# faltiska/Matcha-TTS-24k

Measured on AMD Instinct MI355X. Metric: mel-frames/s (100-bin, 24 kHz) end-to-end synthesise(), n_timesteps=10, higher is better.
Workload: dtype f32 via 2-term f16 split (fp32 accumulate)

## Files before the change

### include/mtts.h

```cpp
#ifndef MTTS_H
#define MTTS_H

#include <stddef.h>
#include <stdint.h>

#ifdef __cplusplus
extern "C" {
#endif

#define MTTS_ABI_VERSION 2
#define MTTS_IMAGE_REVISION 5

typedef struct mtts_ctx mtts_ctx;

typedef struct mtts_config {
    int32_t n_feats;
    int32_t n_spks;
    int32_t spk_emb_dim;
    int32_t n_vocab;
    int32_t enc_channels;
    int32_t enc_filter;
    int32_t enc_heads;
    int32_t enc_layers;
    int32_t enc_kernel;
// ... 60 lines not shown

int mtts_fold_rows(mtts_ctx* ctx, int y_max, int align);
int mtts_cfm_solve_folded(mtts_ctx* ctx, const float* d_x0, const float* d_mu, const int64_t* d_y_lengths, int y_max, int add_mu,
                          const float* h_t_span, int n_steps, int solver, int B, int T, int T_fold, float* d_out, int T_out,
                          float out_scale, float out_shift, void* d_ws, int64_t ws_bytes, void* stream);


int64_t mtts_gemm_packed_bytes(int N, int C, int ntaps);
int mtts_gemm_f32(const float* d_a, int lda, int B, int T_in, int C, int ntaps, const int* h_tap_off, int in_stride,
                  int T_out, const float* d_a_mask, const float* d_a_mean, const float* d_a_rstd, const float* d_a_part,
                  int a_nparts, const float* d_w,
                  void* d_wpacked, const float* d_bias, int N, int act, const float* d_p0, const float* d_p1,
                  const float* d_res, int ldr, const float* d_out_mask, float out_scale, float* d_out, int ldc,
                  float* d_stats_out, int terms, void* stream);

int64_t mtts_gemm_p16_scratch_bytes(int B, int T_in, int C, int T_out, int N);
int mtts_gemm_p16(const float* d_a, int lda, int B, int T_in, int C, int ntaps, const int* h_tap_off, int in_stride, int T_out,
                  const float* d_a_mask, const float* d_a_mean, const float* d_a_rstd, const float* d_a_part, int a_nparts,
                  const float* d_w, void* d_wpacked, const float* d_bias, int N, int act, const float* d_p0, const float* d_p1,
                  const float* d_res, int ldr, const float* d_out_mask, float out_scale, float* d_out, int ldc,
                  float* d_out16_f32, float out_lscale, float* d_stats_out, int force_bm, void* d_scratch, void* stream);

int64_t mtts_conv_gn_scratch_bytes(int B, int T, int C, int N);
int mtts_conv_gn(const float* d_x, int B, int T, int C, int c1, const float* d_w, void* d_wpacked, const float* d_bias, int N,
                 const float* d_gamma, const float* d_beta, const float* d_mask, const float* d_chbias, const int* d_nrows,
                 const int* d_nextra, const float* d_bias_stats, float eps, float* d_out, void* d_scratch, void* stream);

int mtts_attention_f32(const float* d_qkv, const float* d_mask, int B, int T, int H, int D, float scale, int mask_mode,
                       float* d_out, void* stream);

int mtts_attention_p16(const float* d_qkv, const float* d_mask, int B, int T, int H, int D, float scale, int mask_mode,
                       float* d_out, void* d_scratch, void* stream);

int64_t mtts_chain_stream_frags(int C, int inner, int ch, int n_qkv);
int mtts_chain_plan(int M, int ch, int* qb, int* prefetch_wgs);
int mtts_chain_stream_pack(int C, int inner, int ch, int n_qkv, const float* h_w_out, const float* h_w1, const float* h_w2,
                           const float* h_w_qkv, uint16_t* h_dst);
int64_t mtts_chain_stream_frags_pair(int C, int inner, int ch, int n_qkv);
int mtts_chain_stream_pack_pair(int C, int inner, int ch, int n_qkv, const float* h_w_out, const float* h_w1, const float* h_w2,
                                const float* h_w_qkv, uint16_t* h_dst);
int64_t mtts_tblock_chain_scratch_bytes(int M, int C, int inner, int n_qkv, int ch);
int mtts_tblock_chain(const float* d_att, const float* d_x, int M, int C, int inner, const float* h_w_out, const float* h_b_out,
                      const float* h_w1, const float* h_b1, const float* h_p0, const float* h_p1, const float* h_w2,
                      const float* h_b2, const float* h_w_qkv, const float* h_b_qkv, int n_qkv, const float* d_out_mask, int qb,
                      int ch, float* d_x_out, float* d_qkv_out, void* d_scratch, void* stream);
int mtts_tblock_chain_timed(const float* d_att, const float* d_x, int M, int C, int inner, const float* h_w_out, const float* h_b_out,
                            const float* h_w1, const float* h_b1, const float* h_p0, const float* h_p1, const float* h_w2,
                            const float* h_b2, const float* h_w_qkv, const float* h_b_qkv, int n_qkv, const float* d_out_mask,
                            int qb, int ch, float* d_x_out, float* d_qkv_out, void* d_scratch, void* stream, int repeat, float* h_ms);
int mtts_tblock_chain_pair_timed(const float* d_att, const float* d_x, int M, int C, int inner, const float* h_w_out, const float* h_b_out,
                                 const float* h_w1, const float* h_b1, const float* h_p0, const float* h_p1, const float* h_w2,
                                 const float* h_b2, const float* h_w_qkv, const float* h_b_qkv, int n_qkv, const float* d_out_mask,
                                 int qb, int ch, float* d_x_out, float* d_qkv_out, void* d_scratch, void* stream, int repeat, float* h_ms);

int mtts_row_stats(const float* d_x, int M, int C, int ld, float eps, float* d_mean, float* d_rstd, void* stream);

int mtts_channel_layernorm(const float* d_x, int B, int T, int C, const float* d_gamma, const float* d_beta, float eps, int act,
                           const float* d_film, const float* d_mask, float* d_y, void* stream);

int64_t mtts_groupnorm_scratch_bytes(int B, int T, int G);
int mtts_groupnorm_mish(const float* d_y, const float* d_gamma, const float* d_beta, const float* d_mask, int B, int T,
                        int C, int G, float eps, float* d_out, void* d_scratch, void* stream);


typedef struct mtts_vocos mtts_vocos;
mtts_vocos* mtts_vocos_create(int n_mels, int dim, int intermediate_dim, int num_layers, int n_fft, int hop_length);
// ... 26 lines not shown
```

### matcha-tts-24k_amd/_hip.py

```python
from __future__ import annotations

import ctypes as C
import os
import subprocess
from pathlib import Path
from typing import Dict, Optional

import numpy as np
import torch

from .hparams import PathHParams

HERE = Path(__file__).resolve().parent
CSRC = HERE / "csrc"
LIB = Path(os.environ["MTTS_HIP_LIB"]) if os.environ.get("MTTS_HIP_LIB") else HERE / "libmtts_hip.so"
SOURCES = ["gemm_f32.hip", "attention_f32.hip", "gemm_p16.hip", "tblock_chain.hip", "resnet_conv.hip", "norm_glue.hip", "vocos.hip", "model.hip"]
HEADERS = [CSRC / "kernels.h", CSRC / "device_utils.h", CSRC / "model.h", HERE.parent / "include" / "mtts.h"]
SOLVERS = {"euler": 0, "midpoint": 1, "rk4": 2}


class MttsConfig(C.Structure):
    _fields_ = [(n, C.c_int32) for n in (
        "n_feats", "n_spks", "spk_emb_dim", "n_vocab", "enc_channels", "enc_filter", "enc_heads", "enc_layers",
        "enc_kernel", "prenet_layers", "prenet_kernel", "dp_filter", "dp_kernel", "dp_layers", "dec_levels")] + [
        ("dec_channels", C.c_int32 * 4)] + [(n, C.c_int32) for n in (
            "dec_head_dim", "dec_heads", "dec_n_blocks", "dec_mid_blocks")]


def _deps(src: Path, seen=None):
    import re
    seen = set() if seen is None else seen
    if src in seen or not src.exists():
        return seen
    seen.add(src)
    for inc in re.findall(r'^\s*#\s*include\s+"([^"]+)"', src.read_text(), flags=re.M):
        _deps((src.parent / inc).resolve(), seen)
    return seen


BUILD_MODE = "not built in this process"


def build(force: bool = False, verbose: bool = False) -> Path:
    global BUILD_MODE
    srcs = [CSRC / s for s in SOURCES]
    if LIB.exists() and not force:
        deps = set(HEADERS)
        for src in srcs:
            deps |= _deps(src.resolve())
# ... 44 lines not shown
    if _lib is not None:
        return _lib
    if not LIB.exists():
        raise RuntimeError(f"{LIB} is missing: run `python -c 'import __graft_entry__ as g; g.build()'` "
                           "(the HIP path has no CPU fallback)")
    lib = C.CDLL(str(LIB))
    vp, i32, i64, f32 = C.c_void_p, C.c_int, C.c_int64, C.c_float
    sig = {
        "mtts_abi_version": (i32, []),
        "mtts_last_error": (C.c_char_p, []),
        "mtts_create": (vp, [C.POINTER(MttsConfig)]),
        "mtts_destroy": (None, [vp]),
        "mtts_set_tensor": (i32, [vp, C.c_char_p, vp, i64]),
        "mtts_weights_bytes": (i64, [vp]),
        "mtts_upload_weights": (i32, [vp, vp, i64]),
        "mtts_debug_hold": (i32, [vp, i32]),
        "mtts_weights_signature": (i32, [vp, C.c_char_p, i64]),
        "mtts_export_weights": (i32, [vp, vp, i64, C.POINTER(i32)]),
        "mtts_import_weights": (i32, [vp, vp, i64, i32]),
        "mtts_encoder_workspace_bytes": (i64, [vp, i32, i32]),
        "mtts_text_encoder_forward": (i32, [vp, vp, vp, vp, vp, i32, i32, vp, vp, vp, vp, i64, vp]),
        "mtts_speaker_embedding": (i32, [vp, i32, vp, i32, vp, vp]),
        "mtts_durations": (i32, [vp, vp, f32, f32, i32, i32, vp, vp, vp, vp]),
        "mtts_durations_per_utterance": (i32, [vp, vp, vp, vp, i32, i32, vp, vp, vp, vp]),
        "mtts_align_pool": (i32, [vp, vp, vp, i32, i32, i32, i32, vp, vp, vp, vp]),
        "mtts_set_frame_limits": (i32, [vp, vp]),
        "mtts_decoder_workspace_bytes": (i64, [vp, i32, i32]),
        "mtts_decoder_forward": (i32, [vp, vp, vp, vp, f32, i32, i32, vp, vp, i64, vp]),
        "mtts_cfm_solve": (i32, [vp, vp, vp, vp, i32, vp, i32, i32, i32, i32, vp, i32, f32, f32, vp, i64, vp]),
        "mtts_fold_rows": (i32, [vp, i32, i32]),
        "mtts_cfm_solve_folded": (i32, [vp, vp, vp, vp, i32, i32, vp, i32, i32, i32, i32, i32, vp, i32, f32, f32, vp, i64, vp]),
        "mtts_gemm_packed_bytes": (i64, [i32, i32, i32]),
        "mtts_attention_p16": (i32, [vp, vp, i32, i32, i32, i32, f32, i32, vp, vp, vp]),
        "mtts_gemm_p16_scratch_bytes": (i64, [i32, i32, i32, i32, i32]),
        "mtts_conv_gn_scratch_bytes": (i64, [i32, i32, i32, i32]),
        "mtts_conv_gn": (i32, [vp, i32, i32, i32, i32, vp, vp, vp, i32, vp, vp, vp, vp, vp, vp, vp, f32, vp, vp, vp]),
        "mtts_gemm_p16": (i32, [vp, i32, i32, i32, i32, i32, vp, i32, i32, vp, vp, vp, vp, i32, vp, vp, vp, i32, i32, vp, vp, vp,
                                i32, vp, f32, vp, i32, vp, f32, vp, i32, vp, vp]),
        "mtts_gemm_f32": (i32, [vp, i32, i32, i32, i32, i32, vp, i32, i32, vp, vp, vp, vp, i32, vp, vp, vp, i32, i32, vp, vp, vp,
                                i32, vp, f32, vp, i32, vp, i32, vp]),
        "mtts_attention_f32": (i32, [vp, vp, i32, i32, i32, i32, f32, i32, vp, vp]),
        "mtts_chain_stream_frags": (i64, [i32, i32, i32, i32]),
        "mtts_chain_plan": (i32, [i32, i32, C.POINTER(C.c_int), C.POINTER(C.c_int)]),
        "mtts_chain_stream_frags_pair": (i64, [i32, i32, i32, i32]),
        "mtts_chain_stream_pack_pair": (i32, [i32, i32, i32, i32, vp, vp, vp, vp, vp]),
        "mtts_chain_stream_pack": (i32, [i32, i32, i32, i32, vp, vp, vp, vp, vp]),
        "mtts_tblock_chain_scratch_bytes": (i64, [i32, i32, i32, i32, i32]),
        "mtts_tblock_chain": (i32, [vp, vp, i32, i32, i32, vp, vp, vp, vp, vp, vp, vp, vp, vp, vp, i32, vp, i32, i32, vp, vp, vp, vp]),
        "mtts_tblock_chain_timed": (i32, [vp, vp, i32, i32, i32, vp, vp, vp, vp, vp, vp, vp, vp, vp, vp, i32, vp, i32, i32, vp, vp, vp, vp,
                                          i32, C.POINTER(C.c_float)]),
        "mtts_tblock_chain_pair_timed": (i32, [vp, vp, i32, i32, i32, vp, vp, vp, vp, vp, vp, vp, vp, vp, vp, i32, vp, i32, i32, vp, vp, vp, vp,
                                          i32, C.POINTER(C.c_float)]),
        "mtts_row_stats": (i32, [vp, i32, i32, i32, f32, vp, vp, vp]),
        "mtts_channel_layernorm": (i32, [vp, i32, i32, i32, vp, vp, f32, i32, vp, vp, vp, vp]),
        "mtts_groupnorm_scratch_bytes": (i64, [i32, i32, i32]),
        "mtts_groupnorm_mish": (i32, [vp, vp, vp, vp, i32, i32, i32, i32, f32, vp, vp, vp]),
        "mtts_vocos_create": (vp, [i32, i32, i32, i32, i32, i32]),
        "mtts_vocos_destroy": (None, [vp]),
        "mtts_vocos_set_tensor": (i32, [vp, C.c_char_p, vp, i64]),
        "mtts_vocos_weights_bytes": (i64, [vp]),
        "mtts_vocos_upload_weights": (i32, [vp, vp, i64]),
        "mtts_vocos_workspace_bytes": (i64, [vp, i32, i32]),
        "mtts_vocos_decode": (i32, [vp, vp, i32, i32, vp, vp, i64, vp]),
        "mtts_gemm_terms": (i32, [vp]),
        "mtts_set_arithmetic": (i32, [vp, i32]),
        "mtts_weights_saturate": (i32, [vp]),
# ... 389 lines not shown
    n = lib.mtts_tblock_chain_scratch_bytes(M, Cc, inner, n_qkv, ch)
    if n < 0:
        raise RuntimeError("mtts_tblock_chain: unsupported shape")
    scratch = torch.empty(n, dtype=torch.uint8, device=x.device)
    x_out = torch.empty(M, Cc, dtype=torch.float32, device=x.device)
    qkv = torch.empty(M, n_qkv, dtype=torch.float32, device=x.device) if n_qkv else None
    keep = [_host(t) for t in (w_out, b_out, w1, b1, p0, p1, w2, b2, w_qkv, b_qkv)]
    hp = [k[1] for k in keep]
    ms = C.c_float(0.0)
    check((lib.mtts_tblock_chain_pair_timed if pair else lib.mtts_tblock_chain_timed)(ptr(att), ptr(x), M, Cc, inner, hp[0], hp[1], hp[2], hp[3], hp[4], hp[5], hp[6], hp[7], hp[8], hp[9],
                                      n_qkv, ptr(out_mask), qb, ch, ptr(x_out), ptr(qkv), scratch.data_ptr(), stream_ptr(), repeat,
                                      C.byref(ms)))
    torch.cuda.synchronize()
    if repeat:
        return x_out, qkv, ms.value
    return x_out, qkv


def attention_f32(qkv, mask, B, T, H, D, scale, mask_mode):
    lib = load()
    out = torch.empty(B * T, H * D, dtype=torch.float32, device=qkv.device)
    check(lib.mtts_attention_f32(ptr(qkv), ptr(mask), B, T, H, D, float(scale), mask_mode, ptr(out), stream_ptr()))
    return out


def attention_p16(qkv, mask, B, T, H, D, scale, mask_mode):
    lib = load()
    out = torch.empty(B * T, H * D, dtype=torch.float32, device=qkv.device)
    scratch = torch.empty(16 * B * T * H * D, dtype=torch.uint8, device=qkv.device)
    check(lib.mtts_attention_p16(ptr(qkv), ptr(mask), B, T, H, D, float(scale), mask_mode, ptr(out), scratch.data_ptr(), stream_ptr()))
    return out


def row_stats(x, eps=1e-5):
    lib = load()
    M, Cc = x.shape
    mean = torch.empty(M, dtype=torch.float32, device=x.device)
    rstd = torch.empty(M, dtype=torch.float32, device=x.device)
    check(lib.mtts_row_stats(ptr(x), M, Cc, Cc, eps, ptr(mean), ptr(rstd), stream_ptr()))
    return mean, rstd


def channel_layernorm(x, gamma, beta, B, T, *, act=0, film=None, mask=None, eps=1e-5):
    lib = load()
    y = torch.empty_like(x)
    check(lib.mtts_channel_layernorm(ptr(x), B, T, x.shape[1], ptr(gamma), ptr(beta), float(eps), act, ptr(film), ptr(mask), ptr(y),
                                     stream_ptr()))
    return y


def groupnorm_mish(y, gamma, beta, mask, B, T, G=8, eps=1e-5):
    lib = load()
    Cc = y.shape[1]
    scratch = torch.empty(lib.mtts_groupnorm_scratch_bytes(B, T, G), dtype=torch.uint8, device=y.device)
    out = torch.empty_like(y)
    check(lib.mtts_groupnorm_mish(ptr(y), ptr(gamma), ptr(beta), ptr(mask), B, T, Cc, G, eps, ptr(out), scratch.data_ptr(),
                                  stream_ptr()))
    return out
```

### matcha-tts-24k_amd/csrc/attention_f32.hip

```cpp
#include "kernels.h"
#include "device_utils.h"
#include <cstdlib>
#include <string>

namespace mtts {

using f32x16 = __attribute__((ext_vector_type(16))) float;
using f32x4 = __attribute__((ext_vector_type(4))) float;
using f16x8 = __attribute__((ext_vector_type(8))) _Float16;
using f16x4 = __attribute__((ext_vector_type(4))) _Float16;

constexpr int AT_QW = 32;
constexpr int AT_K = 64;
constexpr int AT_D = 64;
constexpr int AT_KS = 72;
constexpr float NEG_BIG = -1e30f;
constexpr float LOG2E = 1.44269504088896340736f;

__device__ __forceinline__ f16x4 tr_read4(const _Float16* lds_ptr) {
    typedef __fp16 h4 __attribute__((__vector_size__(4 * sizeof(__fp16))));
    const h4 v = __builtin_amdgcn_ds_read_tr16_b64_v4f16((__attribute__((address_space(3))) h4*)(lds_ptr));
    return __builtin_bit_cast(f16x4, v);
}

// ... 294 lines not shown
                        *reinterpret_cast<f16x4*>(op + t * 32 + 8 * g4 + 4 * h) = hh;
                    } else {
                        *reinterpret_cast<f16x4*>(op + t * 64 + 8 * g4 + 4 * h) = hh;
                        *reinterpret_cast<f16x4*>(op + t * 64 + 32 + 8 * g4 + 4 * h) = ll;
                    }
                }
        }
        raise_range_flag(p.range_flag, range_bad);
    } else if (q_in) {
        float* op = p.out + (rowbase + qi) * (size_t)(p.H * p.D) + head * p.D;
#pragma unroll
        for (int t = 0; t < 2; ++t)
#pragma unroll
            for (int g4 = 0; g4 < 4; ++g4) {
                const int d = 32 * t + 8 * g4 + 4 * h;
                if (d < p.D) {
                    f32x4 v = {o[t][4 * g4] * inv, o[t][4 * g4 + 1] * inv, o[t][4 * g4 + 2] * inv, o[t][4 * g4 + 3] * inv};
                    *reinterpret_cast<f32x4*>(op + d) = v;
                }
            }
    }
}

hipError_t launch_attention(const AttnArgs& a, hipStream_t s) {
    const bool p16 = a.qkv16 != nullptr;
    const int ew = a.half16 ? 1 : 2;
    if ((a.half16 && !p16) || (a.bf16 && !a.half16)) return hipErrorInvalidValue;
    if (p16 ? (!a.out16 || a.D != AT_D || a.ld16 < 3 * ew * a.H * AT_D || (a.ld16 & 7) || a.ldo16 < ew * a.H * AT_D || (a.ldo16 & 3))
            : (!a.qkv || !a.out))
        return hipErrorInvalidValue;
    if (a.B <= 0 || a.T <= 0 || a.H <= 0) return hipErrorInvalidValue;
    if (a.D <= 0 || a.D > AT_D || (a.D & 3)) return hipErrorInvalidValue;
    if (a.mask_mode == 1 && !a.mask) return hipErrorInvalidValue;
    const int b128 = (a.T + 127) / 128, b64 = (a.T + 63) / 64;
    const long blocks128 = (long)b128 * a.H * a.B;
    const double waste128 = 1.0 - (double)a.T / (b128 * 128.0);
    static const int env_nw = [] { const char* e = getenv("MTTS_ATTN_NW"); return e ? atoi(e) : 0; }();
    const bool same_rows = b128 * 128 == b64 * 64 && blocks128 >= 512;
    const bool use128 = env_nw == 4 || (env_nw == 0 && ((blocks128 >= 768 && waste128 < 0.1) || same_rows));
    {
        static thread_local std::string tag;
        const bool one = a.half16 || (p16 && a.fast16);
        tag = std::string("attention_f32_kernel<") + (use128 ? "4" : "2") + ", " + tf(p16) + ", " + tf(one) + ", " + tf(a.half16) + ", " + tf(a.half16 && a.bf16) + ", 64>";
        g_kernel_tag = tag.c_str();
    }
    static const bool whole_on = [] { const char* e = getenv("MTTS_ATTN_WHOLE"); return !(e && e[0] == '0'); }();
    if (p16 && whole_on && env_nw == 0 && a.T > 64 && a.T <= 192) {
        static thread_local std::string wtag;
        const bool one = a.half16 || a.fast16;
        wtag = std::string("attention_f32_kernel<6, true, ") + tf(one) + ", " + tf(a.half16) + ", " + tf(a.half16 && a.bf16) + ", 192>";
        g_kernel_tag = wtag.c_str();
        const dim3 grid(a.H * a.B), block(384);
        if (a.half16 && a.bf16) hipLaunchKernelGGL((attention_f32_kernel<6, true, true, true, true, 192>), grid, block, 0, s, a);
        else if (a.half16) hipLaunchKernelGGL((attention_f32_kernel<6, true, true, true, false, 192>), grid, block, 0, s, a);
        else if (a.fast16) hipLaunchKernelGGL((attention_f32_kernel<6, true, true, false, false, 192>), grid, block, 0, s, a);
        else hipLaunchKernelGGL((attention_f32_kernel<6, true, false, false, false, 192>), grid, block, 0, s, a);
        return hipGetLastError();
    }
    if (use128) {
        if (a.half16 && a.bf16) hipLaunchKernelGGL((attention_f32_kernel<4, true, true, true, true>), dim3(b128 * a.H * a.B), dim3(256), 0, s, a);
        else if (a.half16) hipLaunchKernelGGL((attention_f32_kernel<4, true, true, true>), dim3(b128 * a.H * a.B), dim3(256), 0, s, a);
        else if (p16 && a.fast16) hipLaunchKernelGGL((attention_f32_kernel<4, true, true>), dim3(b128 * a.H * a.B), dim3(256), 0, s, a);
        else if (p16) hipLaunchKernelGGL((attention_f32_kernel<4, true>), dim3(b128 * a.H * a.B), dim3(256), 0, s, a);
        else hipLaunchKernelGGL((attention_f32_kernel<4, false>), dim3(b128 * a.H * a.B), dim3(256), 0, s, a);
    } else {
        if (a.half16 && a.bf16) hipLaunchKernelGGL((attention_f32_kernel<2, true, true, true, true>), dim3(b64 * a.H * a.B), dim3(128), 0, s, a);
// ... 10 lines not shown
```

### matcha-tts-24k_amd/csrc/kernels.h

```cpp
#pragma once
#include <hip/hip_runtime.h>
#include <stdint.h>
#include <stdlib.h>

namespace mtts {

constexpr int GEMM_BM = 128;
constexpr int GEMM_BN = 128;
constexpr int GEMM_BK = 32;
constexpr int MAX_TAPS = 7;

static inline int round_up(int x, int m) { return (x + m - 1) / m * m; }

extern thread_local const char* g_kernel_tag;
static inline const char* tf(bool b) { return b ? "true" : "false"; }

enum Act { ACT_NONE = 0, ACT_RELU = 1, ACT_SILU = 2, ACT_SNAKE = 3, ACT_GELU = 4 };

struct GemmArgs {
    const float* a0 = nullptr;
    const float* a1 = nullptr;
    int lda0 = 0, lda1 = 0;
    int c0 = 0, c1 = 0;
    int ktap = 0;
// ... 64 lines not shown
}
static inline double gemm_bytes(const GemmArgs& a) {
    const double M = double(a.B) * a.T_out, Min = double(a.B) * a.T_in;
    const double outs = (a.out ? 1.0 : 0.0) + (a.out16 ? 1.0 : 0.0);
    const double ins = ((a.res || a.res16) ? 1.0 : 0.0) + (a.gnr_y ? 1.0 : 0.0);
    return 4.0 * (Min * (a.c0 + a.c1) + double(a.N) * a.ntaps * (a.c0 + a.c1) + M * a.N * (outs + ins));
}

void pack_weight_host(const float* w, int kind, int N, int C, int ntaps, int kT, const int* tsel, const float* col_scale,
                      float* dst, int ktap = 0);
hipError_t launch_pack_weight(const float* w, int N, int C, int ntaps, float* dst, hipStream_t s);
void split_panel_host(const float* panel, size_t n, uint16_t* planes);
hipError_t launch_split_panel(const float* panel, size_t n, void* planes, hipStream_t s);
void split_panel_f16_host(const float* panel, size_t n, uint16_t* planes);
void panel_h16_host(const float* panel, size_t n, uint16_t* plane);
void panel_bf16_host(const float* panel, size_t n, uint16_t* plane);
hipError_t launch_split_panel_f16(const float* panel, size_t n, void* planes, hipStream_t s);

struct AttnArgs {
    const float* qkv = nullptr;
    const float* mask = nullptr;
    float* out = nullptr;
    int B = 0, T = 0, H = 0, D = 0;
    float scale = 1.0f;
    int mask_mode = 0;
    const _Float16* qkv16 = nullptr; int ld16 = 0;
    _Float16* out16 = nullptr; int ldo16 = 0;
    float out_lscale = 2048.0f;
    const int* klen = nullptr;
    bool fast16 = false;
    unsigned int* range_flag = nullptr;
    bool half16 = false;
    bool bf16 = false;
};
hipError_t launch_attention(const AttnArgs& a, hipStream_t s);
static inline double attn_flops(const AttnArgs& a) { return 4.0 * double(a.B) * a.H * double(a.T) * a.T * a.D; }
static inline double attn_bytes(const AttnArgs& a) { return 4.0 * double(a.B) * a.T * 4.0 * a.H * a.D; }

constexpr int CONV_GN_CPG = 48;
constexpr int CONV_GN_MIN_ROWS = 65;
constexpr int CONV_GN_SPLIT_ROWS = 192;
constexpr int CONV_GN_MAX_ROWS = 384;
struct ConvGnArgs {
    const _Float16* a16_0 = nullptr;
    const _Float16* a16_1 = nullptr;
    int lda16_0 = 0, lda16_1 = 0;
    int c0 = 0, c1 = 0;
    const void* w16 = nullptr;
    const float* bias = nullptr;
    int B = 0, T = 0, N = 0;
    const float* gamma = nullptr; const float* beta = nullptr;
    const float* mask = nullptr;
    const float* chbias = nullptr;
    const int* nrows = nullptr;
    const int* nextra = nullptr;
    const float* bias_stats = nullptr;
    float eps = 1e-5f;
    _Float16* out16 = nullptr; int ld16 = 0;
    const float* out16_mask = nullptr;
    unsigned int* range_flag = nullptr;
};
bool conv_gn_supported(int T, int N);
hipError_t launch_conv_gn(const ConvGnArgs& a, hipStream_t s);
static inline double conv_gn_flops(const ConvGnArgs& a) { return 2.0 * double(a.B) * a.T * a.N * 3.0 * (a.c0 + a.c1); }
static inline double conv_gn_bytes(const ConvGnArgs& a) {
    const double M = double(a.B) * a.T, kin = a.c0 + a.c1;
    return 4.0 * (M * kin + double(a.N) * 3.0 * kin + M * a.N);
}
// ... 139 lines not shown
```

### matcha-tts-24k_amd/csrc/model.h

```cpp
#pragma once
#include <atomic>
#include <map>
#include <string>
#include <vector>

#include "../../include/mtts.h"
#include "kernels.h"

namespace mtts {

void set_error(const std::string& msg);
const char* get_error();

struct Panel {
    size_t w = 0, b = 0;
    size_t w16 = 0;
    bool has_bias = false;
    size_t wsum = 0;
    size_t wh16 = 0;
    int N = 0, C = 0, ntaps = 1, ktap = 0;
};
struct Vec { size_t off = 0; int n = 0; };

struct ResnetW {
// ... 41 lines not shown
    Panel dp_proj;
};

struct VocosW {
    Panel embed, head, basis;
    Vec norm_g, norm_b, fin_g, fin_b, window;
    std::vector<Vec> dw_w, dw_b, ln_g, ln_b;
    std::vector<Panel> pw1, pw2;
};

struct ProfRec { hipEvent_t e0, e1; int klass; double flops, bytes; std::string tag; };

}

struct mtts_ctx {
    mtts_config cfg;
    std::map<std::string, std::vector<float>> raw;
    std::vector<float> image;
    float* d_image = nullptr;
    bool packed = false, uploaded = false;
    int gemm_terms = 6;
    unsigned int* cur_flag = nullptr;
    bool weights_saturate = false;
    const int* d_tlen = nullptr;
    bool half16 = false;
    bool bf16 = false;
    bool half_now = false;
    bool fast16 = false;
    bool p16_on = true;
    bool chain_on = true;
    int chain_ch = 256;
    int chain_qb = 0;
    int resnet_fuse = 3;
    int resnet_fuse_rows = mtts::CONV_GN_MAX_ROWS;
    bool pair_on = true;
    unsigned int pair_epoch = 0;
    int chain_min_rows = 5761;
    mtts::DecW dec;
    mtts::EncW enc;
    std::atomic<bool> in_use{false};
    bool prof_on = false;
    std::vector<mtts::ProfRec> prof;
    std::vector<hipEvent_t> ev_pool;
    size_t ev_used = 0;
};

struct mtts_vocos {
    mtts_ctx base;
    int n_mels = 100, dim = 512, inter = 1536, layers = 8, n_fft = 1024, hop = 256;
    int ld_spec = 0, im_off = 0;
    mtts::VocosW w;
};
```

### matcha-tts-24k_amd/csrc/model.hip

```cpp
#include "model.h"

#include <cmath>
#include <cstdlib>
#include <cstring>
#include <time.h>

namespace mtts {

static thread_local std::string g_err;
void set_error(const std::string& m) { g_err = m; }
const char* get_error() { return g_err.c_str(); }

#define HIP_OK(expr)                                                                        \
    do {                                                                                    \
        hipError_t _e = (expr);                                                             \
        if (_e != hipSuccess) {                                                             \
            set_error(std::string(#expr) + ": " + hipGetErrorString(_e));                   \
            return -1;                                                                      \
        }                                                                                   \
    } while (0)
#define RET_IF(expr)          \
    do {                      \
        int _r = (expr);      \
        if (_r) return _r;    \
// ... 11 lines not shown
    c->ev_used += 2;
    HIP_OK(hipEventRecord(r.e0, s));
    c->prof.push_back(r);
    return 0;
}
static int prof_end(mtts_ctx* c, hipStream_t s) {
    if (!c || !c->prof_on) return 0;
    HIP_OK(hipEventRecord(c->prof.back().e1, s));
    c->prof.back().tag = g_kernel_tag ? g_kernel_tag : "";
    return 0;
}
#define LAUNCH(ctx, klass, flops, stream, call)  \
    LAUNCHB(ctx, klass, flops, 0.0, stream, call)
#define LAUNCHB(ctx, klass, flops, bytes, stream, call)  \
    do {                                         \
        RET_IF(prof_begin(ctx, klass, flops, bytes, stream)); \
        HIP_OK(call);                            \
        RET_IF(prof_end(ctx, stream));           \
    } while (0)

static int run_gemm(mtts_ctx* c, const GemmArgs& a0, hipStream_t s) {
    GemmArgs a = a0;
    a.range_flag = c->cur_flag;
    a.half16 = c->half_now && a.a16_0 != nullptr;
    a.bf16 = a.half16 && c->bf16;
    LAUNCHB(c, 0, gemm_flops(a), gemm_bytes(a), s, launch_gemm(a, s));
    return 0;
}
static int run_attn(mtts_ctx* c, const AttnArgs& a0, hipStream_t s) {
    AttnArgs a = a0;
    a.range_flag = c->cur_flag;
    a.half16 = c->half_now && a.qkv16 != nullptr;
    a.bf16 = a.half16 && c->bf16;
    LAUNCHB(c, 1, attn_flops(a), attn_bytes(a), s, launch_attention(a, s));
    return 0;
}
static int chain_prefetch_wgs() {
    static const int n = [] { const char* e = getenv("MTTS_CHAIN_PF"); const int v = e ? atoi(e) : 16; return v < 0 ? 0 : (v > 64 ? 64 : v); }();
    return n;
}
static void chain_plan(int M, int ch, int qb_forced, int* qb, int* pf) {
    const int qb_big = ch == 256 ? 48 : 64, want = chain_prefetch_wgs();
    const bool fits32 = (M + 31) / 32 + want <= 256;
    *qb = (qb_forced == 32 || qb_forced == qb_big) ? qb_forced : (fits32 ? 32 : qb_big);
    const int nwg = (M + *qb - 1) / *qb;
    *pf = want;
    if (nwg <= 256 && nwg + *pf > 256) *pf = (want >= 8 && nwg + 8 <= 256) ? 8 : 0;
}
static int run_chain(mtts_ctx* c, const ChainArgs& a0, hipStream_t s) {
    ChainArgs a = a0;
    a.range_flag = c->cur_flag;
    { int qb_unused = 0; chain_plan(a.M, a.ch, a.qb, &qb_unused, &a.pf_wgs); }
    if (a.pair) a.pf_wgs = chain_prefetch_wgs() ? 16 : 0;
    LAUNCHB(c, 0, chain_flops(a), chain_bytes(a), s, launch_tblock_chain(a, s));
    return 0;
}
#ifdef MTTS_CHAIN_VERIFY
constexpr int VERIFY_SLOTS = 8192;
static int* g_verify = nullptr;
static int g_verify_n = 0;
__global__ void chain_verify_kernel(const uint4* a, const uint4* b, int rows, int cpr, int* out) {
    const long i = (long)blockIdx.x * blockDim.x + threadIdx.x;
    if (i >= (long)rows * cpr) return;
    const uint4 x = a[i], y = b[i];
    if (x.x != y.x || x.y != y.y || x.z != y.z || x.w != y.w) {
        const int row = (int)(i / cpr), ch = (int)(i % cpr);
// ... 1024 lines not shown

using namespace mtts;

extern "C" {

int mtts_abi_version(void) { return MTTS_ABI_VERSION; }
const char* mtts_last_error(void) { return get_error(); }

mtts_ctx* mtts_create(const mtts_config* cfg) {
    if (!cfg) { set_error("null config"); return nullptr; }
    const mtts_config& g = *cfg;
    std::string why;
    if (g.dec_levels < 1 || g.dec_levels > 4) why = "dec_levels must be 1..4";
    else if (g.n_feats <= 0 || (2 * g.n_feats) % 4) why = "n_feats must be even";
    else if ((g.enc_channels + g.spk_emb_dim) % g.enc_heads) why = "encoder hidden size not divisible by heads";
    else if (((g.enc_channels + g.spk_emb_dim) / g.enc_heads) % 4 || (g.enc_channels + g.spk_emb_dim) / g.enc_heads > 64) why = "encoder head dim must be a multiple of 4, <= 64";
    else if (g.dec_head_dim % 4 || g.dec_head_dim > 64) why = "decoder head dim must be a multiple of 4, <= 64";
    else if (g.enc_channels % 4 || g.spk_emb_dim % 4 || g.enc_filter % 4 || g.dp_filter % 4) why = "channel counts must be multiples of 4";
    else if (g.enc_kernel > MAX_TAPS || g.prenet_kernel > MAX_TAPS || g.dp_kernel > MAX_TAPS) why = "kernel sizes above 5 unsupported";
    for (int i = 0; why.empty() && i < g.dec_levels; ++i)
        if (g.dec_channels[i] % 32) why = "decoder channels must be multiples of 32 (8 GroupNorm groups of 4k channels, K segments of 32)";
    if (!why.empty()) { set_error(why); return nullptr; }
    mtts_ctx* c = new mtts_ctx();
    c->cfg = g;
    c->gemm_terms = default_gemm_terms();
    { const char* e = getenv("MTTS_GEMM_TERMS"); c->fast16 = e && atoi(e) == 1; c->half16 = e && (atoi(e) == 16 || atoi(e) == 17); c->bf16 = e && atoi(e) == 17; }
    { const char* e = getenv("MTTS_P16"); c->p16_on = !(e && e[0] == '0'); }
    { const char* e = getenv("MTTS_CHAIN"); c->chain_on = !(e && e[0] == '0'); }
    { const char* e = getenv("MTTS_CHAIN_CH"); c->chain_ch = (e && atoi(e) == 128) ? 128 : 256; }
    { const char* e = getenv("MTTS_CHAIN_QB"); c->chain_qb = e ? atoi(e) : 0; }
    { const char* e = getenv("MTTS_CHAIN_MIN_ROWS"); if (e) c->chain_min_rows = atoi(e); }
    { const char* e = getenv("MTTS_CHAIN_PAIR"); c->pair_on = !(e && e[0] == '0'); }
    { const char* e = getenv("MTTS_RESNET_FUSE"); if (e) c->resnet_fuse = atoi(e) & 7; }
    { const char* e = getenv("MTTS_RESNET_FUSE_ROWS"); if (e) c->resnet_fuse_rows = atoi(e); }
    if (c->pair_on) {
        int dev = 0;
        hipDeviceProp_t prop;
        if (hipGetDevice(&dev) == hipSuccess && hipGetDeviceProperties(&prop, dev) == hipSuccess && prop.multiProcessorCount < 256) c->pair_on = false;
        (void)hipGetLastError();
    }
    return c;
}

int mtts_set_arithmetic(mtts_ctx* c, int terms) {
    if (!c) { set_error("null context"); return -1; }
    if (terms != 0 && terms != 1 && terms != 2 && terms != 3 && terms != 6 && terms != 16 && terms != 17) {
        set_error("mtts_set_arithmetic: terms must be 0, 1, 2, 3, 6, 16 or 17");
        return -1;
    }
    c->fast16 = terms == 1;
    c->half16 = terms == 16 || terms == 17;
    c->bf16 = terms == 17;
    c->gemm_terms = (terms == 1 || terms == 16 || terms == 17) ? 2 : terms;
    c->packed = false;
    c->uploaded = false;
    return 0;
}

int mtts_weights_saturate(mtts_ctx* c) {
    if (!c) { set_error("null context"); return -1; }
    if (!c->packed && pack_all(c)) return -1;
    return c->weights_saturate ? 1 : 0;
}

void mtts_destroy(mtts_ctx* c) {
    if (!c) return;
// ... 469 lines not shown
    if (c1) { a.a16_1 = a16 + 2 * (C - c1); a.lda16_1 = 2 * C; a.c1 = c1; }
    a.w16 = planes; a.bias = d_bias; a.B = B; a.T = T; a.N = N;
    a.gamma = d_gamma; a.beta = d_beta; a.mask = d_mask; a.chbias = d_chbias; a.nrows = d_nrows; a.nextra = d_nextra; a.bias_stats = d_bias_stats;
    a.eps = eps; a.out16 = o16; a.ld16 = 2 * N;
    HIP_OK(launch_conv_gn(a, s));
    HIP_OK(launch_from_p16(o16, 2 * N, B * T, N, 2048.0f, d_out, N, s));
    return 0;
}

int mtts_attention_f32(const float* d_qkv, const float* d_mask, int B, int T, int H, int D, float scale, int mask_mode, float* d_out,
                       void* stream) {
    AttnArgs a;
    a.qkv = d_qkv; a.mask = d_mask; a.out = d_out; a.B = B; a.T = T; a.H = H; a.D = D; a.scale = scale; a.mask_mode = mask_mode;
    HIP_OK(launch_attention(a, static_cast<hipStream_t>(stream)));
    return 0;
}

int mtts_attention_p16(const float* d_qkv, const float* d_mask, int B, int T, int H, int D, float scale, int mask_mode, float* d_out,
                       void* d_scratch, void* stream) {
    hipStream_t s = static_cast<hipStream_t>(stream);
    if (D != 64 || !d_scratch) { set_error("P16 attention needs D == 64 and a scratch buffer"); return -1; }
    const int M = B * T, C3 = 3 * H * D;
    _Float16* q16 = static_cast<_Float16*>(d_scratch);
    _Float16* o16 = q16 + (size_t)M * 2 * C3;
    HIP_OK(launch_to_p16(d_qkv, C3, nullptr, M, C3, C3, q16, 2 * C3, 1.0f, s));
    AttnArgs a;
    a.qkv16 = q16; a.ld16 = 2 * C3; a.out16 = o16; a.ldo16 = 2 * H * D; a.mask = d_mask;
    a.B = B; a.T = T; a.H = H; a.D = D; a.scale = scale; a.mask_mode = mask_mode;
    HIP_OK(launch_attention(a, s));
    HIP_OK(launch_from_p16(o16, 2 * H * D, M, H * D, a.out_lscale, d_out, H * D, s));
    return 0;
}

int mtts_row_stats(const float* d_x, int M, int C, int ld, float eps, float* d_mean, float* d_rstd, void* stream) {
    HIP_OK(launch_row_stats(d_x, M, C, ld, eps, d_mean, d_rstd, static_cast<hipStream_t>(stream)));
    return 0;
}

int mtts_channel_layernorm(const float* d_x, int B, int T, int C, const float* d_gamma, const float* d_beta, float eps, int act,
                           const float* d_film, const float* d_mask, float* d_y, void* stream) {
    if (B <= 0 || T <= 0) { set_error("mtts_channel_layernorm: empty batch"); return -1; }
    if (act != ACT_NONE && act != ACT_SILU) { set_error("mtts_channel_layernorm: act must be 0 (none) or 2 (SiLU)"); return -1; }
    LayerNormArgs a;
    a.x = d_x; a.ldx = C; a.y = d_y; a.ldy = C; a.M = B * T; a.C = C; a.T = T; a.gamma = d_gamma; a.beta = d_beta; a.eps = eps;
    a.act = act; a.film = d_film; a.mask = d_mask;
    HIP_OK(launch_layernorm(a, static_cast<hipStream_t>(stream)));
    return 0;
}

int64_t mtts_groupnorm_scratch_bytes(int B, int T, int G) { return (int64_t)B * gn_chunks_max(T) * G * 2 * (int64_t)sizeof(float); }

int mtts_groupnorm_mish(const float* d_y, const float* d_gamma, const float* d_beta, const float* d_mask, int B, int T, int C, int G,
                        float eps, float* d_out, void* d_scratch, void* stream) {
    hipStream_t s = static_cast<hipStream_t>(stream);
    HIP_OK(launch_gn_partial(d_y, B, T, C, G, static_cast<float*>(d_scratch), s));
    GnApplyArgs a;
    a.y = d_y; a.partial = static_cast<const float*>(d_scratch); a.gamma = d_gamma; a.beta = d_beta; a.mask = d_mask;
    a.out = d_out; a.B = B; a.T = T; a.C = C; a.G = G; a.eps = eps;
    HIP_OK(launch_gn_apply(a, s));
    return 0;
}

int mtts_chain_plan(int M, int ch, int* qb, int* prefetch_wgs) {
    if (M <= 0 || (ch != 128 && ch != 256) || !qb || !prefetch_wgs) { set_error("mtts_chain_plan: bad argument"); return -1; }
    chain_plan(M, ch, 0, qb, prefetch_wgs);
    return 0;
// ... 373 lines not shown
```

Before: 431,500.

## Add DMA-staged MFMA flash attention kernel for p16 split-f16 path

Adds a new flash-attention kernel for the 2-term f16 split path. It streams K/V tiles straight from global memory into a double-buffered LDS ring with global_load_lds, reads V through transposed ds_read_b64_tr_b16, and uses 32x32x16 MFMAs with an online softmax. launch_attention now routes to this kernel by default whenever the inputs qualify (D=64, no mask_mode, T between 65 and 2048), choosing 4 or 6 waves per block by sequence length. It also honours per-batch key lengths so padded keys can be skipped. The aim is to overlap key/value loads with compute and cut register and LDS staging overhead, at the cost of new hand-written asm paths with numerical and correctness risk.

```diff
diff --git a/include/mtts.h b/include/mtts.h
--- a/include/mtts.h
+++ b/include/mtts.h
@@ -116,6 +116,9 @@
 int mtts_attention_p16(const float* d_qkv, const float* d_mask, int B, int T, int H, int D, float scale, int mask_mode,
                        float* d_out, void* d_scratch, void* stream);
 
+int mtts_attention_p16_variant(const float* d_qkv, const float* d_mask, const int* d_klen, int B, int T, int H, int D,
+                               float scale, int mask_mode, int variant, float* d_out, void* d_scratch, void* stream);
+
 int64_t mtts_chain_stream_frags(int C, int inner, int ch, int n_qkv);
 int mtts_chain_plan(int M, int ch, int* qb, int* prefetch_wgs);
 int mtts_chain_stream_pack(int C, int inner, int ch, int n_qkv, const float* h_w_out, const float* h_w1, const float* h_w2,
diff --git a/matcha-tts-24k_amd/_hip.py b/matcha-tts-24k_amd/_hip.py
--- a/matcha-tts-24k_amd/_hip.py
+++ b/matcha-tts-24k_amd/_hip.py
@@ -14,7 +14,7 @@
 HERE = Path(__file__).resolve().parent
 CSRC = HERE / "csrc"
 LIB = Path(os.environ["MTTS_HIP_LIB"]) if os.environ.get("MTTS_HIP_LIB") else HERE / "libmtts_hip.so"
-SOURCES = ["gemm_f32.hip", "attention_f32.hip", "gemm_p16.hip", "tblock_chain.hip", "resnet_conv.hip", "norm_glue.hip", "vocos.hip", "model.hip"]
+SOURCES = ["gemm_f32.hip", "attention_f32.hip", "attention_p16.hip", "gemm_p16.hip", "tblock_chain.hip", "resnet_conv.hip", "norm_glue.hip", "vocos.hip", "model.hip"]
 HEADERS = [CSRC / "kernels.h", CSRC / "device_utils.h", CSRC / "model.h", HERE.parent / "include" / "mtts.h"]
 SOLVERS = {"euler": 0, "midpoint": 1, "rk4": 2}
 
@@ -125,6 +125,7 @@
         "mtts_cfm_solve_folded": (i32, [vp, vp, vp, vp, i32, i32, vp, i32, i32, i32, i32, i32, vp, i32, f32, f32, vp, i64, vp]),
         "mtts_gemm_packed_bytes": (i64, [i32, i32, i32]),
         "mtts_attention_p16": (i32, [vp, vp, i32, i32, i32, i32, f32, i32, vp, vp, vp]),
+        "mtts_attention_p16_variant": (i32, [vp, vp, vp, i32, i32, i32, i32, f32, i32, i32, vp, vp, vp]),
         "mtts_gemm_p16_scratch_bytes": (i64, [i32, i32, i32, i32, i32]),
         "mtts_conv_gn_scratch_bytes": (i64, [i32, i32, i32, i32]),
         "mtts_conv_gn": (i32, [vp, i32, i32, i32, i32, vp, vp, vp, i32, vp, vp, vp, vp, vp, vp, vp, f32, vp, vp, vp]),
@@ -580,6 +581,15 @@
     return out
 
 
+def attention_p16_variant(qkv, mask, B, T, H, D, scale, variant, klen=None, mask_mode=0):
+    lib = load()
+    out = torch.empty(B * T, H * D, dtype=torch.float32, device=qkv.device)
+    scratch = torch.empty(16 * B * T * H * D, dtype=torch.uint8, device=qkv.device)
+    check(lib.mtts_attention_p16_variant(ptr(qkv), ptr(mask), ptr(klen) if klen is not None else None, B, T, H, D, float(scale),
+                                         mask_mode, variant, ptr(out), scratch.data_ptr(), stream_ptr()))
+    return out
+
+
 def row_stats(x, eps=1e-5):
     lib = load()
     M, Cc = x.shape
diff --git a/matcha-tts-24k_amd/csrc/attention_f32.hip b/matcha-tts-24k_amd/csrc/attention_f32.hip
--- a/matcha-tts-24k_amd/csrc/attention_f32.hip
+++ b/matcha-tts-24k_amd/csrc/attention_f32.hip
@@ -350,6 +350,7 @@
     if (a.B <= 0 || a.T <= 0 || a.H <= 0) return hipErrorInvalidValue;
     if (a.D <= 0 || a.D > AT_D || (a.D & 3)) return hipErrorInvalidValue;
     if (a.mask_mode == 1 && !a.mask) return hipErrorInvalidValue;
+    if (a.dma && attention_p16_supported(a) && (a.dma & (a.T <= 192 ? 2 : 1))) return launch_attention_p16(a, s);
     const int b128 = (a.T + 127) / 128, b64 = (a.T + 63) / 64;
     const long blocks128 = (long)b128 * a.H * a.B;
     const double waste128 = 1.0 - (double)a.T / (b128 * 128.0);
diff --git a/matcha-tts-24k_amd/csrc/attention_p16.hip b/matcha-tts-24k_amd/csrc/attention_p16.hip
--- /dev/null
+++ b/matcha-tts-24k_amd/csrc/attention_p16.hip
@@ -0,0 +1,278 @@
+#include "kernels.h"
+#include "device_utils.h"
+
+namespace mtts {
+
+using f32x16 = __attribute__((ext_vector_type(16))) float;
+using f32x4 = __attribute__((ext_vector_type(4))) float;
+using f16x8 = __attribute__((ext_vector_type(8))) _Float16;
+using f16x4 = __attribute__((ext_vector_type(4))) _Float16;
+
+constexpr int AP_QW = 32;
+constexpr int AP_K = 64;
+constexpr int AP_D = 64;
+constexpr int AP_KBYTES = AP_K * 256;
+constexpr int AP_STAGE = 2 * AP_KBYTES;
+constexpr int AP_PIECES = AP_STAGE / 1024;
+constexpr int AP_OS = 272;
+constexpr int AP_LDS = 2 * AP_STAGE + ATTN_DMA_MAXKEYS * 4;
+constexpr float AP_NEG_BIG = -1e30f;
+constexpr float AP_LOG2E = 1.44269504088896340736f;
+static_assert(AP_PIECES == 32, "16 K pieces + 16 V pieces");
+
+#define MTTS_AP_GLDS16(gp, lp) \
+    __builtin_amdgcn_global_load_lds((const __attribute__((address_space(1))) void*)(gp), (__attribute__((address_space(3))) void*)(lp), 16, 0, 0)
+
+using u32x2 = __attribute__((ext_vector_type(2))) unsigned int;
+template <int OFF>
+__device__ __forceinline__ void ap_v_reads(u32x2 (&r)[8], unsigned addr) {
+    asm volatile(
+        "ds_read_b64_tr_b16 %0, %8 offset:%9\n\tds_read_b64_tr_b16 %1, %8 offset:%10\n\t"
+        "ds_read_b64_tr_b16 %2, %8 offset:%11\n\tds_read_b64_tr_b16 %3, %8 offset:%12\n\t"
+        "ds_read_b64_tr_b16 %4, %8 offset:%13\n\tds_read_b64_tr_b16 %5, %8 offset:%14\n\t"
+        "ds_read_b64_tr_b16 %6, %8 offset:%15\n\tds_read_b64_tr_b16 %7, %8 offset:%16"
+        : "=&v"(r[0]), "=&v"(r[1]), "=&v"(r[2]), "=&v"(r[3]), "=&v"(r[4]), "=&v"(r[5]), "=&v"(r[6]), "=&v"(r[7])
+        : "v"(addr), "n"(OFF), "n"(OFF + 512), "n"(OFF + 8192), "n"(OFF + 8192 + 512), "n"(OFF + 4096), "n"(OFF + 4096 + 512),
+          "n"(OFF + 4096 + 8192), "n"(OFF + 4096 + 8192 + 512)
+        : "memory");
+}
+template <int N>
+__device__ __forceinline__ void ap_v_wait(u32x2 (&r)[8]) {
+    asm volatile("s_waitcnt lgkmcnt(%8)" : "+v"(r[0]), "+v"(r[1]), "+v"(r[2]), "+v"(r[3]), "+v"(r[4]), "+v"(r[5]), "+v"(r[6]), "+v"(r[7]) : "n"(N));
+}
+__device__ __forceinline__ f16x8 ap_join(u32x2 a, u32x2 b) {
+    using u32x4 = __attribute__((ext_vector_type(4))) unsigned int;
+    return __builtin_bit_cast(f16x8, u32x4{a[0], a[1], b[0], b[1]});
+}
+
+__device__ __forceinline__ void ap_wait_barrier() { asm volatile("s_waitcnt vmcnt(0) lgkmcnt(0)\n\ts_barrier" ::: "memory"); }
+
+template <int SUBS>
+__device__ __forceinline__ void ap_tile(const char* st, unsigned st_lds, const float* Bs, const f16x8 (&qh)[4], const f16x8 (&ql)[4], f32x16 (&o)[2],
+                                        float& m_run, float& l_run, float scale2, unsigned kaddr, int lane) {
+    const int h = lane >> 5;
+    f32x16 s[SUBS];
+#pragma unroll
+    for (int t = 0; t < SUBS; ++t) {
+#pragma unroll
+        for (int r = 0; r < 16; ++r) s[t][r] = 0.f;
+#pragma unroll
+        for (int kb = 0; kb < 4; ++kb) {
+            const unsigned cc = (kb >> 1) * 8 + (kb & 1) * 2;
+            const f16x8 kh = *reinterpret_cast<const f16x8*>(st + (kaddr ^ (cc << 4)) + t * (32 * 256));
+            const f16x8 kl = *reinterpret_cast<const f16x8*>(st + (kaddr ^ ((cc + 4) << 4)) + t * (32 * 256));
+            s[t] = __builtin_amdgcn_mfma_f32_32x32x16_f16(kl, qh[kb], s[t], 0, 0, 0);
+            s[t] = __builtin_amdgcn_mfma_f32_32x32x16_f16(kh, ql[kb], s[t], 0, 0, 0);
+            s[t] = __builtin_amdgcn_mfma_f32_32x32x16_f16(kh, qh[kb], s[t], 0, 0, 0);
+        }
+    }
+    float mx = AP_NEG_BIG;
+#pragma unroll
+    for (int t = 0; t < SUBS; ++t)
+#pragma unroll
+        for (int g4 = 0; g4 < 4; ++g4) {
+            const f32x4 bb = *reinterpret_cast<const f32x4*>(Bs + 32 * t + 8 * g4 + 4 * h);
+#pragma unroll
+            for (int e = 0; e < 4; ++e) {
+                const float v = fmaf(s[t][4 * g4 + e], scale2, bb[e]);
+                s[t][4 * g4 + e] = v;
+                mx = fmaxf(mx, v);
+            }
+        }
+    mx = fmaxf(mx, __shfl_xor(mx, 32));
+    const float m_new = fmaxf(m_run, mx);
+    const float alpha = __builtin_amdgcn_exp2f(m_run - m_new);
+    float psum = 0.f;
+#pragma unroll
+    for (int t = 0; t < SUBS; ++t)
+#pragma unroll
+        for (int r = 0; r < 16; ++r) {
+            const float pv = __builtin_amdgcn_exp2f(s[t][r] - m_new);
+            s[t][r] = pv;
+            psum += pv;
+        }
+    l_run = l_run * alpha + psum;
+    if (__any(m_new != m_run)) {
+#pragma unroll
+        for (int t = 0; t < 2; ++t)
+#pragma unroll
+            for (int r = 0; r < 16; ++r) o[t][r] *= alpha;
+    }
+    m_run = m_new;
+    const unsigned va = st_lds + AP_KBYTES + (4 * h + ((lane & 15) >> 2)) * 64 + 32 * ((lane >> 4) & 1) + 8 * (lane & 3);
+    u32x2 vr[2][8];
+    ap_v_reads<0>(vr[0], va);
+#pragma unroll
+    for (int g = 0; g < 2 * SUBS; ++g) {
+        const int t = g >> 1, ks = g & 1;
+        if (g == 0) ap_v_reads<1024>(vr[1], va);
+        if (g == 1 && SUBS == 2) ap_v_reads<2048>(vr[0], va);
+        if (g == 2) ap_v_reads<3072>(vr[1], va);
+        f16x8 ph, pl;
+#pragma unroll
+        for (int j = 0; j < 8; ++j) {
+            const float pv = s[t][8 * ks + j];
+            const _Float16 a = (_Float16)pv;
+            ph[j] = a;
+            pl[j] = (_Float16)(pv - (float)a);
+        }
+        if (g + 1 < 2 * SUBS) ap_v_wait<8>(vr[g & 1]);
+        else ap_v_wait<0>(vr[g & 1]);
+#pragma unroll
+        for (int dt = 0; dt < 2; ++dt) {
+            const f16x8 vh = ap_join(vr[g & 1][4 * dt], vr[g & 1][4 * dt + 1]), vl = ap_join(vr[g & 1][4 * dt + 2], vr[g & 1][4 * dt + 3]);
+            o[dt] = __builtin_amdgcn_mfma_f32_32x32x16_f16(vl, ph, o[dt], 0, 0, 0);
+            o[dt] = __builtin_amdgcn_mfma_f32_32x32x16_f16(vh, pl, o[dt], 0, 0, 0);
+            o[dt] = __builtin_amdgcn_mfma_f32_32x32x16_f16(vh, ph, o[dt], 0, 0, 0);
+        }
+    }
+}
+
+template <int NW>
+__global__ __launch_bounds__(64 * NW, NW == 6 ? 3 : 2) void attention_p16_kernel(const AttnArgs p) {
+    constexpr int NT = 64 * NW;
+    constexpr int PW = (AP_PIECES + NW - 1) / NW;
+    static_assert(NW * AP_QW * AP_OS <= 2 * AP_STAGE, "the parked O tiles overlay the ring");
+    extern __shared__ __attribute__((aligned(16))) char ap_lds[];
+    float* Bs = reinterpret_cast<float*>(ap_lds + 2 * AP_STAGE);
+    const unsigned lds0 = (unsigned)(uintptr_t)(__attribute__((address_space(3))) char*)ap_lds;
+
+    const int tid = threadIdx.x, lane = tid & 63, wave = __builtin_amdgcn_readfirstlane(tid >> 6);
+    const int lq = lane & 31, h = lane >> 5;
+    const int qblocks = (p.T + NW * AP_QW - 1) / (NW * AP_QW);
+    int swz;
+    {
+        const int nwg = gridDim.x, id = blockIdx.x;
+        const int xcd = id & 7, q = nwg >> 3, r = nwg & 7;
+        swz = (xcd < r ? xcd * (q + 1) : r * (q + 1) + (xcd - r) * q) + (id >> 3);
+    }
+    const int qb = swz % qblocks, head = (swz / qblocks) % p.H, b = swz / (qblocks * p.H);
+    const int q0 = qb * (NW * AP_QW) + wave * AP_QW;
+    const size_t rowbase = (size_t)b * p.T;
+    const int Tb = p.klen ? min(p.T, p.klen[b]) : p.T;
+    const int ntiles = (Tb + AP_K - 1) / AP_K;
+    const int rem = Tb - (ntiles - 1) * AP_K;
+    const int nloop = (ntiles > 0 && rem <= 32) ? ntiles - 1 : ntiles;
+    const float ninf = -__builtin_huge_valf();
+    const _Float16* q16 = p.qkv16 + head * (2 * AP_D);
+    const _Float16* kv16 = q16 + 2 * p.H * AP_D + rowbase * (size_t)p.ld16;
+
+    const int kq = lane >> 4, vq = lane >> 2;
+    const unsigned ksrc = ((lane & 15) ^ kq) << 3, vsrc = 2 * p.H * AP_D + ((lane & 3) << 3);
+    auto issue = [&](int kt) {
+        char* st = ap_lds + (kt & 1) * AP_STAGE;
+#pragma unroll
+        for (int i = 0; i < PW; ++i) {
+            const int pc = wave + NW * i;
+            if (AP_PIECES % NW == 0 || i + 1 < PW || pc < AP_PIECES) {
+                const bool isv = pc >= AP_PIECES / 2;
+                const int pv = pc - AP_PIECES / 2, rg = pv >> 2;
+                const int key = min(kt * AP_K + (isv ? 16 * (pv & 3) + vq : 4 * pc + kq), Tb - 1);
+                const unsigned src = isv ? vsrc + (((rg & 1) * 2 + (rg >> 1)) << 5) : ksrc ^ ((pc & 3) << 5);
+                MTTS_AP_GLDS16(kv16 + ((unsigned)key * (unsigned)p.ld16 + src), st + pc * 1024);
+            }
+        }
+    };
+    if (ntiles > 0) issue(0);
+
+    const int qi = q0 + lq;
+    const bool q_in = qi < p.T;
+    const float scale2 = p.scale * AP_LOG2E;
+    f16x8 qh[4], ql[4];
+    {
+        const _Float16* qrow = q16 + (rowbase + (q_in ? qi : 0)) * (size_t)p.ld16;
+#pragma unroll
+        for (int kb = 0; kb < 4; ++kb) {
+            const f16x8 z = {0, 0, 0, 0, 0, 0, 0, 0};
+            const _Float16* src = qrow + (kb >> 1) * 64 + (kb & 1) * 16 + 8 * h;
+            qh[kb] = q_in ? *reinterpret_cast<const f16x8*>(src) : z;
+            ql[kb] = q_in ? *reinterpret_cast<const f16x8*>(src + 32) : z;
+        }
+    }
+    for (int k = tid; k < ntiles * AP_K; k += NT) {
+        float bv = ninf;
+        if (k < Tb) bv = (p.mask ? p.mask[rowbase + k] : 1.0f) * AP_LOG2E;
+        Bs[k] = bv;
+    }
+
+    f32x16 o[2];
+#pragma unroll
+    for (int t = 0; t < 2; ++t)
+#pragma unroll
+        for (int r = 0; r < 16; ++r) o[t][r] = 0.f;
+    float m_run = AP_NEG_BIG, l_run = 0.f;
+    const unsigned kaddr = lq * 256 + (((lq & 15) ^ h) << 4);
+
+    const bool active = q0 < p.T;
+    for (int kt = 0; kt < nloop; ++kt) {
+        ap_wait_barrier();
+        if (kt + 1 < ntiles) issue(kt + 1);
+        if (active) ap_tile<2>(ap_lds + (kt & 1) * AP_STAGE, lds0 + (kt & 1) * AP_STAGE, Bs + kt * AP_K, qh, ql, o, m_run, l_run, scale2, kaddr, lane);
+    }
+    if (nloop < ntiles) {
+        ap_wait_barrier();
+        if (active) ap_tile<1>(ap_lds + (nloop & 1) * AP_STAGE, lds0 + (nloop & 1) * AP_STAGE, Bs + nloop * AP_K, qh, ql, o, m_run, l_run, scale2, kaddr, lane);
+    }
+
+    const float l_tot = l_run + __shfl_xor(l_run, 32);
+    const float inv = l_tot > 0.f ? 1.0f / l_tot : 0.f;
+    bool range_bad = false;
+    asm volatile("s_waitcnt lgkmcnt(0)\n\ts_barrier" ::: "memory");
+    char* ot = ap_lds + wave * (AP_QW * AP_OS);
+#pragma unroll
+    for (int t = 0; t < 2; ++t)
+#pragma unroll
+        for (int g4 = 0; g4 < 4; ++g4) {
+            f16x4 hh, ll;
+            if (q_in) range_bad |= out_of_f16_range(o[t][4 * g4] * inv, o[t][4 * g4 + 1] * inv, o[t][4 * g4 + 2] * inv, o[t][4 * g4 + 3] * inv);
+#pragma unroll
+            for (int e = 0; e < 4; ++e) {
+                _Float16 a, c;
+                split_f16(o[t][4 * g4 + e] * inv, p.out_lscale, a, c);
+                hh[e] = a;
+                ll[e] = c;
+            }
+            *reinterpret_cast<f16x4*>(ot + lq * AP_OS + (t * 64 + 8 * g4 + 4 * h) * 2) = hh;
+            *reinterpret_cast<f16x4*>(ot + lq * AP_OS + (t * 64 + 32 + 8 * g4 + 4 * h) * 2) = ll;
+        }
+    raise_range_flag(p.range_flag, range_bad);
+    asm volatile("s_waitcnt lgkmcnt(0)" ::: "memory");
+    __builtin_amdgcn_wave_barrier();
+    _Float16* obase = p.out16 + rowbase * (size_t)p.ldo16 + head * (2 * AP_D);
+#pragma unroll
+    for (int i = 0; i < 8; ++i) {
+        const int qr = 4 * i + (lane >> 4), row = q0 + qr;
+        const f32x4 v = *reinterpret_cast<const f32x4*>(ot + qr * AP_OS + (lane & 15) * 16);
+        if (row < p.T) *reinterpret_cast<f32x4*>(obase + (size_t)row * p.ldo16 + (lane & 15) * 8) = v;
+    }
+}
+
+bool attention_p16_supported(const AttnArgs& a) {
+    return a.qkv16 && a.out16 && !a.half16 && !a.fast16 && a.D == AP_D && a.mask_mode == 0 && a.T <= ATTN_DMA_MAXKEYS &&
+           !(a.ld16 & 7) && !(a.ldo16 & 7) && a.B > 0 && a.T > AP_K && a.H > 0;
+}
+
+template <int NW>
+static hipError_t ap_launch(const AttnArgs& a, hipStream_t s) {
+    static bool configured = false;
+    if (!configured) {
+        hipError_t e = hipFuncSetAttribute(reinterpret_cast<const void*>(attention_p16_kernel<NW>), hipFuncAttributeMaxDynamicSharedMemorySize, AP_LDS);
+        if (e != hipSuccess) return e;
+        configured = true;
+    }
+    const int qblocks = (a.T + NW * AP_QW - 1) / (NW * AP_QW);
+    hipLaunchKernelGGL(attention_p16_kernel<NW>, dim3(qblocks * a.H * a.B), dim3(64 * NW), AP_LDS, s, a);
+    return hipGetLastError();
+}
+
+hipError_t launch_attention_p16(const AttnArgs& a, hipStream_t s) {
+    if (!attention_p16_supported(a)) return hipErrorInvalidValue;
+    if (a.T > 192) {
+        g_kernel_tag = "attention_p16_kernel<4>";
+        return ap_launch<4>(a, s);
+    }
+    g_kernel_tag = "attention_p16_kernel<6>";
+    return ap_launch<6>(a, s);
+}
+
+}
diff --git a/matcha-tts-24k_amd/csrc/kernels.h b/matcha-tts-24k_amd/csrc/kernels.h
--- a/matcha-tts-24k_amd/csrc/kernels.h
+++ b/matcha-tts-24k_amd/csrc/kernels.h
@@ -120,8 +120,12 @@
     unsigned int* range_flag = nullptr;
     bool half16 = false;
     bool bf16 = false;
+    int dma = 3;
 };
 hipError_t launch_attention(const AttnArgs& a, hipStream_t s);
+constexpr int ATTN_DMA_MAXKEYS = 2048;
+bool attention_p16_supported(const AttnArgs& a);
+hipError_t launch_attention_p16(const AttnArgs& a, hipStream_t s);
 static inline double attn_flops(const AttnArgs& a) { return 4.0 * double(a.B) * a.H * double(a.T) * a.T * a.D; }
 static inline double attn_bytes(const AttnArgs& a) { return 4.0 * double(a.B) * a.T * 4.0 * a.H * a.D; }
 
diff --git a/matcha-tts-24k_amd/csrc/model.h b/matcha-tts-24k_amd/csrc/model.h
--- a/matcha-tts-24k_amd/csrc/model.h
+++ b/matcha-tts-24k_amd/csrc/model.h
@@ -97,6 +97,7 @@
     int chain_ch = 256;
     int chain_qb = 0;
     int resnet_fuse = 3;
+    int attn_dma = 3;
     int resnet_fuse_rows = mtts::CONV_GN_MAX_ROWS;
     bool pair_on = true;
     unsigned int pair_epoch = 0;
diff --git a/matcha-tts-24k_amd/csrc/model.hip b/matcha-tts-24k_amd/csrc/model.hip
--- a/matcha-tts-24k_amd/csrc/model.hip
+++ b/matcha-tts-24k_amd/csrc/model.hip
@@ -67,6 +67,7 @@
     a.range_flag = c->cur_flag;
     a.half16 = c->half_now && a.qkv16 != nullptr;
     a.bf16 = a.half16 && c->bf16;
+    a.dma = c->attn_dma;
     LAUNCHB(c, 1, attn_flops(a), attn_bytes(a), s, launch_attention(a, s));
     return 0;
 }
@@ -1157,6 +1158,7 @@
     { const char* e = getenv("MTTS_CHAIN_MIN_ROWS"); if (e) c->chain_min_rows = atoi(e); }
     { const char* e = getenv("MTTS_CHAIN_PAIR"); c->pair_on = !(e && e[0] == '0'); }
     { const char* e = getenv("MTTS_RESNET_FUSE"); if (e) c->resnet_fuse = atoi(e) & 7; }
+    { const char* e = getenv("MTTS_ATTN_DMA"); if (e) c->attn_dma = atoi(e) & 3; }
     { const char* e = getenv("MTTS_RESNET_FUSE_ROWS"); if (e) c->resnet_fuse_rows = atoi(e); }
     if (c->pair_on) {
         int dev = 0;
@@ -1692,6 +1694,22 @@
     return 0;
 }
 
+int mtts_attention_p16_variant(const float* d_qkv, const float* d_mask, const int* d_klen, int B, int T, int H, int D, float scale,
+                               int mask_mode, int variant, float* d_out, void* d_scratch, void* stream) {
+    hipStream_t s = static_cast<hipStream_t>(stream);
+    if (D != 64 || !d_scratch) { set_error("P16 attention needs D == 64 and a scratch buffer"); return -1; }
+    const int M = B * T, C3 = 3 * H * D;
+    _Float16* q16 = static_cast<_Float16*>(d_scratch);
+    _Float16* o16 = q16 + (size_t)M * 2 * C3;
+    HIP_OK(launch_to_p16(d_qkv, C3, nullptr, M, C3, C3, q16, 2 * C3, 1.0f, s));
+    AttnArgs a;
+    a.qkv16 = q16; a.ld16 = 2 * C3; a.out16 = o16; a.ldo16 = 2 * H * D; a.mask = d_mask; a.klen = d_klen;
+    a.B = B; a.T = T; a.H = H; a.D = D; a.scale = scale; a.mask_mode = mask_mode; a.dma = variant & 3;
+    HIP_OK(launch_attention(a, s));
+    HIP_OK(launch_from_p16(o16, 2 * H * D, M, H * D, a.out_lscale, d_out, H * D, s));
+    return 0;
+}
+
 int mtts_row_stats(const float* d_x, int M, int C, int ld, float eps, float* d_mean, float* d_rstd, void* stream) {
     HIP_OK(launch_row_stats(d_x, M, C, ld, eps, d_mean, d_rstd, static_cast<hipStream_t>(stream)));
     return 0;
```

Result: no change. 434,300, median of 6 (+0.7%).
